# wangrui2025/GDKVM

Hardware: AMD Instinct MI355X
Metric: frames/sec (GDKVM forward + argmax mask), EchoNet 112x112x32 clips (higher is better)
Workload: dtype bf16; 1 GPU; BASELINE.json configs[1]: EchoNet-Dynamic 112x112x32 bf16 inference, batch=16 per GPU; clips_per_gpu=16, frames_per_clip=32, image=112x112, heads=1, key_dim=64, rule=delta_sequential, world_size=1, ranks_seen=1

## Files before the change

### gdkvm_amd/csrc/conv3x3_tile.hip

```cpp
#include <atomic>
#include "gdkvm_device.hpp"

namespace {

constexpr int CT_CK = 64;
constexpr int CT_PIX = 160;
constexpr int CT_SLOTS = CT_PIX / 16;
constexpr int CT_MAXMT = 13;
constexpr int CT_VARIANT_128 = 4, CT_VARIANT_64 = 3;

struct ConvTileArgs {
    const bf16_t* x; const bf16_t* w; const float* bias; const bf16_t* res; bf16_t* y;
    const bf16_t* x2; int C1;
    int N, H, W, C, K;
    int fpt, th, tiles_y, ntiles;
    int bw, bh, band_px, npieces;
    int relu;
    float inv_band, inv_bw, inv_tw, inv_w;
    int perm;
};

__host__ __device__ __forceinline__ int ct_channel(int kt, int j, int perm)
{
    return perm ? 32 * (kt >> 1) + 8 * (j >> 2) + 4 * (kt & 1) + (j & 3) : 16 * kt + j;
}

template <int NWN, int NTW, bool PK, int NWV = 8, int MAXMT = CT_MAXMT>
__global__ __launch_bounds__(64 * NWV, (NWV == 4 ? 2 : 1)) void conv3x3_tile_kernel(ConvTileArgs a)
{
    constexpr int MW = NWV / NWN, MTW = (MAXMT + MW - 1) / MW;
    extern __shared__ __attribute__((aligned(16))) unsigned char ct_band[];
    const int tid = threadIdx.x, lane = tid & 63, li = lane & 15, g = lane >> 4;
    const int w = __builtin_amdgcn_readfirstlane(tid >> 6), wn = w % NWN, wm = w / NWN;
    const int H = a.H, W = a.W, C = a.C, K = a.K, BW = a.bw;
    const int band_bytes = a.npieces * 1024, nchunk = C / CT_CK;
    const int tpix = a.fpt * a.th * W;
    const int co0 = blockIdx.y * (16 * NTW * NWN) + 16 * NTW * wn;

    f32x4 bias4[NTW];
#pragma unroll
    for (int nt = 0; nt < NTW; ++nt) {
        const int kt = min(co0 / 16 + nt, K / 16 - 1);
        const float* bp = a.bias + ct_channel(kt, 4 * g, a.perm);
        asm volatile("global_load_dwordx4 %0, %1, off" : "=&v"(bias4[nt]) : "v"(bp) : "memory");
    }

    constexpr int PP = NWV == 8 ? 7 : 8;
    const int cs1 = a.C1, cs2 = a.x2 ? C - a.C1 : C;
    unsigned g_off1[PP], g_off2[PP];
#pragma unroll
    for (int u = 0; u < PP; ++u) {
        const int j = w + NWV * u, d = 64 * j + lane, pix = d / CT_SLOTS, c = d - CT_SLOTS * pix;
        const int f = idx_div(pix, a.inv_band), r = pix - f * (a.bh * BW), by = idx_div(r, a.inv_bw), bx = r - by * BW;
        const int sp = (f * H + by - 1) * W + bx - 1;
        const bool live = j < a.npieces && c < 8 && pix < a.band_px && bx >= 1 && bx <= W && (a.tiles_y > 1 || (by >= 1 && by <= a.th));
        g_off1[u] = live ? (unsigned)(sp * cs1 * 2 + c * 16) : RSRC_DEAD;
        g_off2[u] = live ? (unsigned)(sp * cs2 * 2 + c * 16) : RSRC_DEAD;
    }
    const unsigned lds0 = (unsigned)reinterpret_cast<uintptr_t>(ct_band);
    const int nlive = max(0, (a.npieces - w + NWV - 1) / NWV);
    struct Geo { int px0, npx, row0; };
    auto geo_of = [&](int tile) __attribute__((always_inline)) {
        const int ty = tile % a.tiles_y, fg = tile / a.tiles_y;
        Geo q;
        q.px0 = fg * a.fpt * H * W;
        q.npx = min(a.fpt, a.N - fg * a.fpt) * H * W;
        q.row0 = ty * a.th * W;
        return q;
    };
    auto fetch = [&](const Geo q, int chunk, int buf) __attribute__((always_inline)) {
        const bool second = a.x2 != nullptr && chunk * CT_CK >= a.C1;
        const int cs = second ? cs2 : cs1;
        const bf16_t* base = (second ? a.x2 : a.x) + (long long)q.px0 * cs;
        const __amdgpu_buffer_rsrc_t rsrc = make_rsrc(base, q.npx * cs * 2);
        const unsigned ts = (unsigned)((q.row0 * cs + chunk * CT_CK - (second ? a.C1 : 0)) * 2);
        const unsigned dst0 = lds0 + buf * band_bytes + 1024 * w;
#pragma unroll
        for (int u = 0; u < PP; ++u) {
            const unsigned dst = u < nlive ? dst0 + 1024 * NWV * u : lds0 + 2 * band_bytes;
            __builtin_amdgcn_raw_ptr_buffer_load_lds(rsrc, lds_dma_dst(dst), 16,
                                                     (int)((second ? g_off2[u] : g_off1[u]) + ts), 0, 0, 0);
        }
    };

    int tile = blockIdx.x;
    Geo cur = geo_of(min(tile, a.ntiles - 1));
    if (tile < a.ntiles) fetch(cur, 0, 0);

    unsigned pbase[MTW];
#pragma unroll
    for (int m = 0; m < MTW; ++m) {
        const int p = min(16 * (wm + MW * m) + li, tpix - 1);
        const int f = idx_div(p, a.inv_tw), r = p - f * (a.th * W), py = idx_div(r, a.inv_w), px = r - py * W;
        pbase[m] = (unsigned)(((f * a.bh + py) * BW + px) * CT_PIX + g * 16);
    }
    const bf16_t* wrow[NTW];
// ... 27 lines not shown
    constexpr int WD = 3, KU = 6;
    WF wr[WD];
#pragma unroll
    for (int j = 0; j < WD; ++j) wload(wr[j], j);
    for (; tile < a.ntiles; tile += gridDim.x) {
        const Geo nxt = geo_of(min(tile + (int)gridDim.x, a.ntiles - 1));
        f32x4 acc[MTW][NTW];
#pragma unroll
        for (int m = 0; m < MTW; ++m)
#pragma unroll
            for (int nt = 0; nt < NTW; ++nt) acc[m][nt] = f32x4{0.f, 0.f, 0.f, 0.f};
        for (int chunk = 0; chunk < nchunk; ++chunk, ++gc) {
            const int buf = gc & 1;
            asm volatile("s_waitcnt vmcnt(%0) lgkmcnt(0)" ::"n"(WD * NTW) : "memory");
            asm volatile("s_barrier" ::: "memory");
            {
                const bool more = chunk + 1 < nchunk;
                Geo q;
                q.px0 = more ? cur.px0 : nxt.px0; q.npx = more ? cur.npx : nxt.npx; q.row0 = more ? cur.row0 : nxt.row0;
                fetch(q, more ? chunk + 1 : 0, buf ^ 1);
            }
            const unsigned char* band = ct_band + buf * band_bytes;
            auto load_x = [&](bf16x8 (&xb)[MTW], int r) __attribute__((always_inline)) {
                r = min(r, 17);
                const int tap = r >> 1, kh = r & 1, dy = tap / 3, dx = tap - 3 * dy;
                const unsigned off = (unsigned)((dy * BW + dx) * CT_PIX + kh * 64);
#pragma unroll
                for (int m = 0; m < MTW; ++m) {
                    xb[m] = *reinterpret_cast<const bf16x8*>(band + pbase[m] + off);
                }
            };
            auto mfmas = [&](const bf16x8 (&xb)[MTW], const WF& wfr) __attribute__((always_inline)) {
#pragma unroll
                for (int m = 0; m < MTW; ++m)
// ... 218 lines not shown
}

namespace {
template <int NWN, int NTW, int NWV = 8, int MAXMT = CT_MAXMT>
void launch_tile(bool packed, dim3 grid, size_t lds, hipStream_t st, const ConvTileArgs& a)
{
    if (packed) hipLaunchKernelGGL((conv3x3_tile_kernel<NWN, NTW, true, NWV, MAXMT>), grid, dim3(64 * NWV), lds, st, a);
    else hipLaunchKernelGGL((conv3x3_tile_kernel<NWN, NTW, false, NWV, MAXMT>), grid, dim3(64 * NWV), lds, st, a);
}
template <int NWN, int NTW, int NWV = 8, int MAXMT = CT_MAXMT>
bool setattr_tile()
{
    return hipFuncSetAttribute(reinterpret_cast<const void*>(conv3x3_tile_kernel<NWN, NTW, true, NWV, MAXMT>), hipFuncAttributeMaxDynamicSharedMemorySize, 113 * 1024) == hipSuccess
        && hipFuncSetAttribute(reinterpret_cast<const void*>(conv3x3_tile_kernel<NWN, NTW, false, NWV, MAXMT>), hipFuncAttributeMaxDynamicSharedMemorySize, 113 * 1024) == hipSuccess;
}
}

int gdkvm_conv3x3_tile_launch(const void* x, const void* x2, int C1, const void* w, const float* bias, const void* residual, void* y,
                              int N, int C, int H, int W, int K, int relu, int variant, int packed, hipStream_t st)
{
    if (variant == 0 && K % 128 == 0 && CT_VARIANT_128 == 4) {
        if (gdkvm_conv3x3_tile_launch(x, x2, C1, w, bias, residual, y, N, C, H, W, K, relu, 4, packed, st) == 0) return 0;
        variant = 2;
    }
    if (variant == 0 && K % 128 != 0 && (H * W <= 16 * 7 || 2 * W <= 16 * 7)) {
        if (gdkvm_conv3x3_tile_launch(x, x2, C1, w, bias, residual, y, N, C, H, W, K, relu, 5, packed, st) == 0) return 0;
        variant = 3;
    }
    if (C % CT_CK || K % 16 || W > 64 || W < 1 || H < 1 || N < 1 || variant < 0 || variant > 5) return 1;
    if (variant == 4 && K % 128) return 1;
    const bool half = variant == 4 || variant == 5;
    if (x2 && (C1 <= 0 || C1 >= C || C1 % CT_CK)) return 1;
    ConvTileArgs a;
    a.x2 = static_cast<const bf16_t*>(x2); a.C1 = x2 ? C1 : C;
    a.x = static_cast<const bf16_t*>(x); a.w = static_cast<const bf16_t*>(w); a.bias = bias;
    a.res = static_cast<const bf16_t*>(residual); a.y = static_cast<bf16_t*>(y);
    a.N = N; a.H = H; a.W = W; a.C = C; a.K = K; a.relu = relu;
    const int maxpix = half ? 16 * 7 : 16 * CT_MAXMT;
    const int maxpieces = half ? 32 : 56;
    if (H * W <= maxpix) { a.th = H; a.fpt = maxpix / (H * W); a.tiles_y = 1; if (a.fpt > N) a.fpt = N; }
    else { a.fpt = 1; a.th = maxpix / W; if (a.th < 1) return 1; a.tiles_y = (H + a.th - 1) / a.th; }
    a.bw = W + 2; a.bh = a.th + 2;
    auto pieces = [&]() { a.band_px = a.fpt * a.bh * a.bw; return (a.band_px * CT_SLOTS + 63) / 64; };
    while (pieces() > maxpieces && a.fpt > 1) --a.fpt;
    while (pieces() > maxpieces && a.th > 1) { --a.th; a.bh = a.th + 2; a.tiles_y = (H + a.th - 1) / a.th; }
    a.npieces = pieces();
    if (a.npieces > maxpieces) return 1;
    if ((long long)(a.fpt * H + 2) * W * (x2 ? (C1 > C - C1 ? C1 : C - C1) : C) * 2 >= 0x7fffffffLL) return 1;
    a.inv_band = 1.0f / (float)(a.bh * a.bw); a.inv_bw = 1.0f / (float)a.bw;
    a.inv_tw = 1.0f / (float)(a.th * W); a.inv_w = 1.0f / (float)W;
    a.perm = K % 32 == 0;
    const long long groups = (N + a.fpt - 1) / a.fpt;
    const long long ntiles = groups * a.tiles_y;
    if (ntiles <= 0 || ntiles > 0x7fffffffLL) return 1;
    a.ntiles = (int)ntiles;
    if (variant == 0) variant = K % 128 == 0 ? 2 : CT_VARIANT_64;
    const int kwg = (variant == 2 || variant == 4) ? 128 : 64;
    const int gy = (K + kwg - 1) / kwg;
    const size_t lds = (size_t)2 * a.npieces * 1024 + 1024;
    int per = (half ? 512 : 256) / gy; if (per < 1) per = 1;
    const int gx = (int)(ntiles < per ? ntiles : per);
    static std::atomic<unsigned long long> done_mask{0};
    int dev = 0;
    if (hipGetDevice(&dev) != hipSuccess) return 1;
    const unsigned long long bit = 1ull << (dev & 63);
    if (!(done_mask.load(std::memory_order_relaxed) & bit)) {
        if (!setattr_tile<4, 1>() || !setattr_tile<4, 2>() || !setattr_tile<2, 2>() || !setattr_tile<4, 2, 4, 7>() || !setattr_tile<2, 2, 4, 7>()) return 1;
        done_mask.fetch_or(bit, std::memory_order_relaxed);
    }
    switch (variant) {
// ... 9 lines not shown
```

### gdkvm_amd/csrc/conv_dispatch.hip

```cpp
#include "gdkvm_common.hpp"

int gdkvm_conv3x3_c64_launch(const void* x, const void* w, const float* bias, const void* residual, void* y, int N, int H, int W,
                             int relu, int packed, hipStream_t st);
int gdkvm_conv3x3_tile_launch(const void* x, const void* x2, int C1, const void* w, const float* bias, const void* residual, void* y,
                              int N, int C, int H, int W, int K, int relu, int variant, int packed, hipStream_t st);
int gdkvm_conv_igemm_launch(const void* x, const void* wpacked, const float* bias, const void* residual, void* y,
                            int N, int C, int H, int W, int K, int R, int S, int stride, int pad, int relu,
                            const void* w2packed, const float* bias2, void* y2, hipStream_t st);

extern "C" int gdkvm_conv_bias_act(const void* x, const void* w, const float* bias, const void* residual, void* y,
                                   int N, int C, int H, int W, int K, int R, int S, int stride, int pad, int relu, int kernel,
                                   int io_dtype, void* stream)
{
    if (io_dtype != GDKVM_BF16) return gdkvm_fail(GDKVM_ERR_DTYPE, "conv_bias_act: only bf16 is implemented");
    if (N < 0 || C <= 0 || H <= 0 || W <= 0 || K <= 0 || R <= 0 || S <= 0 || stride <= 0 || pad < 0 || C % 8 || K % 8
        || H + 2 * pad < R || W + 2 * pad < S)
        return gdkvm_fail(GDKVM_ERR_SHAPE, "conv_bias_act: N=%d C=%d H=%d W=%d K=%d %dx%d stride %d pad %d (C, K multiples of 8)",
                          N, C, H, W, K, R, S, stride, pad);
    const bool packed = kernel & GDKVM_CONV_PACKED_WEIGHTS;
    kernel &= ~GDKVM_CONV_PACKED_WEIGHTS;
    if (kernel != 0 && (kernel < 4 || kernel > 11)) return gdkvm_fail(GDKVM_ERR_ARG, "conv_bias_act: kernel=%d (0 = by shape, 4, 5, 6..8, 9, 10, 11)", kernel);
    if (kernel == 9) {
        if (!packed) return gdkvm_fail(GDKVM_ERR_ARG, "conv_bias_act: kernel 9 reads the gdkvm_conv_igemm_pack_weights copy of the weights (flag %d)", GDKVM_CONV_PACKED_WEIGHTS);
        if (C % 32 || K % 128) return gdkvm_fail(GDKVM_ERR_SHAPE, "conv_bias_act: kernel 9 needs C a multiple of 32 and K of 128 (C=%d K=%d)", C, K);
// ... 45 lines not shown
        return gdkvm_fail(GDKVM_ERR_SHAPE, "conv_cat_bias_act: N=%d C1=%d C2=%d H=%d W=%d K=%d (C1, C2 multiples of 64, K of 16)", N, C1, C2, H, W, K);
    if (N == 0) return GDKVM_OK;
    if (!x1 || !x2 || !w || !bias || !y) return gdkvm_fail(GDKVM_ERR_ARG, "conv_cat_bias_act: null pointer");
    if (!gdkvm_aligned16(x1) || !gdkvm_aligned16(x2) || !gdkvm_aligned16(w) || !gdkvm_aligned16(y) || !gdkvm_aligned16(bias) || (residual && !gdkvm_aligned16(residual)))
        return gdkvm_fail(GDKVM_ERR_ARG, "conv_cat_bias_act: pointers must be 16-byte aligned");
    if ((size_t)N * H * W * (C1 + C2) >= (1ull << 31) || (size_t)N * H * W * K >= (1ull << 31))
        return gdkvm_fail(GDKVM_ERR_SHAPE, "conv_cat_bias_act: tensor too large for 32-bit offsets");
    if (int rc = gdkvm_check_device()) return rc;
    if (gdkvm_conv3x3_tile_launch(x1, x2, C1, w, bias, residual, y, N, C1 + C2, H, W, K, relu, kernel >= 10 ? kernel - 6 : (kernel >= 6 ? kernel - 5 : 0), packed ? 1 : 0,
                                  static_cast<hipStream_t>(stream)))
        return gdkvm_fail(GDKVM_ERR_SHAPE, "conv_cat_bias_act: %dx%d is not served (rows of at most 64 pixels)", H, W);
    GDKVM_LAUNCH_CHECK("conv3x3_tile_kernel");
    return GDKVM_OK;
}

extern "C" int gdkvm_conv_down_bias_act(const void* x, const void* w, const float* bias, void* y, int relu,
                                        const void* w_down, const float* bias_down, void* y_down,
                                        int N, int C, int H, int W, int K, int R, int S, int stride, int pad, int io_dtype, void* stream)
{
    if (io_dtype != GDKVM_BF16) return gdkvm_fail(GDKVM_ERR_DTYPE, "conv_down_bias_act: only bf16 is implemented");
    if (N < 0 || C <= 0 || H <= 0 || W <= 0 || K <= 0 || R <= 0 || S != R || !(R & 1) || stride <= 0 || pad != R / 2 || C % 32 || K % 128)
        return gdkvm_fail(GDKVM_ERR_SHAPE, "conv_down_bias_act: N=%d C=%d H=%d W=%d K=%d %dx%d stride %d pad %d (odd square window, pad = R/2, "
                                           "C a multiple of 32, K of 128)", N, C, H, W, K, R, S, stride, pad);
    if (N == 0) return GDKVM_OK;
    if (!x || !w || !bias || !y || !w_down || !y_down) return gdkvm_fail(GDKVM_ERR_ARG, "conv_down_bias_act: null pointer");
    const void* ptrs[] = {x, w, bias, y, w_down, y_down};
    for (const void* p : ptrs) if (!gdkvm_aligned16(p)) return gdkvm_fail(GDKVM_ERR_ARG, "conv_down_bias_act: pointers must be 16-byte aligned");
    if (bias_down && !gdkvm_aligned16(bias_down)) return gdkvm_fail(GDKVM_ERR_ARG, "conv_down_bias_act: pointers must be 16-byte aligned");
    if (int rc = gdkvm_check_device()) return rc;
    if (gdkvm_conv_igemm_launch(x, w, bias, nullptr, y, N, C, H, W, K, R, S, stride, pad, relu, w_down, bias_down, y_down, static_cast<hipStream_t>(stream)))
// ... 5 lines not shown
```

### gdkvm_amd/csrc/gdkvm_device.hpp

```cpp
#pragma once
#include <type_traits>

#include "gdkvm_common.hpp"

typedef float f32x2 __attribute__((ext_vector_type(2)));
typedef unsigned u32x4 __attribute__((ext_vector_type(4)));

template <int I, int E, class F>
__device__ __forceinline__ void static_for(F&& f)
{
    if constexpr (I < E) {
        f(std::integral_constant<int, I>{});
        static_for<I + 1, E>(f);
    }
}

__device__ __forceinline__ int idx_div(int n, float inv) { return (int)(((float)n + 0.5f) * inv); }

__device__ __forceinline__ unsigned pack_bf16x2(float a, float b) { return (unsigned)f32_to_bf16(a) | ((unsigned)f32_to_bf16(b) << 16); }
__device__ __forceinline__ uint2 pack_bf16x4(const f32x4& v) { return make_uint2(pack_bf16x2(v[0], v[1]), pack_bf16x2(v[2], v[3])); }
__device__ __forceinline__ uint4 pack_bf16x8(const float (&v)[8])
{
    uint4 o;
    o.x = pack_bf16x2(v[0], v[1]);
// ... 12 lines not shown
    const unsigned w[4] = {u.x, u.y, u.z, u.w};
#pragma unroll
    for (int j = 0; j < 4; ++j) { v[2 * j] = bf16_lo(w[j]); v[2 * j + 1] = bf16_hi(w[j]); }
}

typedef __attribute__((address_space(3))) void* lds_dst_t;
__device__ __forceinline__ lds_dst_t lds_dma_dst(const void* p) { return reinterpret_cast<lds_dst_t>(reinterpret_cast<uintptr_t>(p)); }
__device__ __forceinline__ lds_dst_t lds_dma_dst(unsigned addr) { return reinterpret_cast<lds_dst_t>(static_cast<uintptr_t>(addr)); }

constexpr int RSRC_WORD3 = 0x00020000;
__device__ __forceinline__ __amdgpu_buffer_rsrc_t make_rsrc(const void* p, int bytes)
{
    return __builtin_amdgcn_make_buffer_rsrc(const_cast<void*>(p), 0, bytes, RSRC_WORD3);
}
constexpr unsigned RSRC_DEAD = 0x80000000u;
```

### gdkvm_amd/model.py

```python
from __future__ import annotations

from dataclasses import dataclass
import os
from typing import NamedTuple, Optional, Tuple

import torch
import torch.nn as nn
import torch.nn.functional as F

from . import ops

_RULES = {"gated_linear": ops.RULE_GATED_LINEAR, "delta_parallel": ops.RULE_DELTA_PARALLEL,
          "delta_sequential": ops.RULE_DELTA_SEQUENTIAL}

_KEY_REMAP: dict = {}


@dataclass
class GDKVMConfig:
    in_channels: int = 3
    num_classes: int = 2
    heads: int = 1
    key_dim: int = 64
    value_dim: int = 256
# ... 223 lines not shown
    buf = torch.empty((x.shape[0], padded), dtype=x.dtype, device=x.device)
    buf[:, :n].copy_(x.reshape(x.shape[0], n))
    return buf[:, :n].unflatten(1, x.shape[1:]) if x.dim() > 2 else buf[:, :n]


class UpBlock(nn.Module):
    def __init__(self, cin, cskip, cout):
        super().__init__()
        self.conv = nn.Sequential(nn.Conv2d(cin + cskip, cout, 3, 1, 1, bias=False), _bn(cout), nn.ReLU(inplace=True),
                                  nn.Conv2d(cout, cout, 3, 1, 1, bias=False), _bn(cout), nn.ReLU(inplace=True))

    def forward(self, x, skip):
        c = self.conv
        if (isinstance(c[0], FusedConv) and not torch.is_grad_enabled() and x.is_cuda and x.dtype == torch.bfloat16
                and skip.dtype == torch.bfloat16 and c[0].cat_served(x.shape[1], skip.shape[1], skip.shape[-1])):
            u = ops.upsample_bilinear(x.contiguous(memory_format=torch.channels_last), skip.shape[2:])
            y = c[0].forward_cat(u, skip)
            for m in list(c)[1:]:
                y = m(y)
            return y
        if (x.is_cuda and x.dtype == torch.bfloat16 and skip.dtype == torch.bfloat16
                and x.shape[1] % 8 == 0 and skip.shape[1] % 8 == 0):
            x = ops.upsample_cat(x.contiguous(memory_format=torch.channels_last),
                                 skip.contiguous(memory_format=torch.channels_last))
        else:
            x = torch.cat([F.interpolate(x, size=skip.shape[-2:], mode="bilinear", align_corners=False), skip], 1)
        if len(c) == 6 and isinstance(c[1], nn.BatchNorm2d):
            return _bn_act(c[4], _conv(c[3], _bn_act(c[1], _conv(c[0], x), True)), True)
        return c(x)


class HeadFeature(NamedTuple):
# ... 74 lines not shown
                and d.conv.out_channels == cv.out_channels and cv.in_channels % 32 == 0 and cv.out_channels % 128 == 0
                and cv.weight.dtype == torch.bfloat16 and d.conv.weight.dtype == torch.bfloat16
                and cv.weight.is_contiguous(memory_format=torch.channels_last)
                and self._tile(cv.in_channels, cv.out_channels, cv.stride[0], False, x.shape[-1]) is None):
            return None
        dw = d.conv.weight if d.conv.weight.is_contiguous(memory_format=torch.channels_last) else d.conv.weight.contiguous(memory_format=torch.channels_last)
        return ops.conv_down_bias_act(x.contiguous(memory_format=torch.channels_last), cv.weight, self.epi.bias, self._packed(x.device, igemm=True),
                                      dw, d._packed(x.device, igemm=True), None, cv.stride[0], self.relu)

    def cat_served(self, c1: int, c2: int, width: int) -> bool:
        cv = self.conv
        return (not getattr(self, "bias_folded_downstream", False) and cv.kernel_size == (3, 3) and cv.groups == 1
                and cv.dilation == (1, 1) and cv.stride == (1, 1) and cv.padding == (1, 1) and cv.weight.is_cuda
                and cv.weight.dtype == torch.bfloat16 and cv.weight.is_contiguous(memory_format=torch.channels_last)
                and c1 % 64 == 0 and c2 % 64 == 0 and c1 + c2 == cv.in_channels and cv.out_channels % 16 == 0 and width <= 64)

    def forward_cat(self, x1, x2):
        cl = torch.channels_last
        return ops.conv_cat_bias_act(x1.contiguous(memory_format=cl), x2.contiguous(memory_format=cl), self.conv.weight, self.epi.bias,
                                     None, self.relu, 0, self._packed(x1.device))

    def forward(self, x, residual=None):
        cv = self.conv
        folded = getattr(self, "bias_folded_downstream", False)
        if (not folded and x.is_cuda and x.dtype == torch.bfloat16 and cv.kernel_size == (3, 3) and cv.groups == 1
                and cv.dilation == (1, 1) and cv.stride[0] == cv.stride[1] and cv.padding == (1, 1) and cv.weight.dtype == torch.bfloat16
                and cv.in_channels % 8 == 0 and cv.out_channels % 8 == 0 and cv.weight.is_contiguous(memory_format=torch.channels_last)):
            tile = self._tile(cv.in_channels, cv.out_channels, cv.stride[0], residual is not None, x.shape[-1])
            if tile is not None:
                packed = self._packed(x.device) if tile in (4, 5) else None
# ... 810 lines not shown
```

### gdkvm_amd/ops.py

```python
from __future__ import annotations

import contextlib
import ctypes
import math
import os
from typing import Optional, Tuple

import torch

RULE_GATED_LINEAR, RULE_DELTA_PARALLEL, RULE_DELTA_SEQUENTIAL = 0, 1, 2
FLAG_NORMALIZE_QK, FLAG_GATE_LOGITS, FLAG_TRAIN, FLAG_WIDE_RANGE = 1, 2, 4, 8


def recurrence_flags(rule: int, flags: int) -> int:
    return flags | FLAG_WIDE_RANGE if rule == RULE_DELTA_PARALLEL else flags
F32, BF16 = 0, 1

_PKG = os.path.dirname(os.path.abspath(__file__))
_SO = os.path.join(_PKG, "libgdkvm_hip.so")
_lib = None
_vp, _sz, _i = ctypes.c_void_p, ctypes.c_size_t, ctypes.c_int

SIGNATURES = {
    "gdkvm_abi_version": (_i, []),
# ... 42 lines not shown
    "gdkvm_head_bwd": (_i, [_vp] * 7 + [_sz] + [_i] * 6 + [_vp]),
    "gdkvm_proj_rows": (_i, [_vp] * 6 + [ctypes.c_longlong] + [_i] * 5 + [_vp]),
    "gdkvm_stem_conv_pool": (_i, [_vp] * 4 + [_i] * 4 + [_vp]),
    "gdkvm_stem_conv_pool_nchw": (_i, [_vp] * 4 + [_i] * 5 + [_vp]),
    "gdkvm_stem_conv_nchw": (_i, [_vp] * 3 + [_i] * 5 + [_vp]),
    "gdkvm_stem_pack_s2d": (_i, [_vp, _vp, _i] + [ctypes.c_longlong] * 4 + [_vp]),
    "gdkvm_stem_wgrad_workspace_bytes": (_sz, [_i] * 3),
    "gdkvm_stem_wgrad_nchw": (_i, [_vp] * 3 + [ctypes.c_longlong] * 4 + [_vp, _sz] + [_i] * 5 + [_vp]),
    "gdkvm_gate_logits": (_i, [_vp] * 7 + [_i] * 5 + [_vp]),
    "gdkvm_proj_gates": (_i, [_vp] * 13 + [_i] * 7 + [_vp]),
    "gdkvm_conv_bias_act": (_i, [_vp] * 5 + [_i] * 12 + [_vp]),
    "gdkvm_conv3x3_pack_weights": (_i, [_vp, _vp, _i, _i, _i, _vp]),
    "gdkvm_conv_igemm_pack_weights": (_i, [_vp, _vp, _i, _i, _i, _i, _i, _vp]),
    "gdkvm_conv_down_bias_act": (_i, [_vp] * 4 + [_i] + [_vp] * 3 + [_i] * 10 + [_vp]),
    "gdkvm_conv_cat_bias_act": (_i, [_vp] * 6 + [_i] * 9 + [_vp]),
    "gdkvm_conv_s2_dgrad_pack_bytes": (_sz, [_i] * 3),
    "gdkvm_conv_s2_pack_train": (_i, [_vp] * 7 + [_i, _i, _vp]),
    "gdkvm_conv_s2_dgrad": (_i, [_vp] * 4 + [_i] * 7 + [_vp]),
    "gdkvm_conv_wgrad_strided_workspace_bytes": (_sz, [_i] * 9),
    "gdkvm_conv_wgrad_strided": (_i, [_vp] * 3 + [ctypes.c_longlong] * 4 + [_vp, _sz] + [_i] * 10 + [_vp]),
    "gdkvm_conv3x3_pack_weights_dgrad": (_i, [_vp, _vp, _i, _i, _i, _vp]),
    "gdkvm_conv3x3_pack_weights_train": (_i, [_i, _vp, _vp, _vp, _vp, _vp, _vp, _vp]),
    "gdkvm_conv3x3_wgrad_workspace_bytes": (_sz, [_i] * 5),
    "gdkvm_conv3x3_wgrad": (_i, [_vp, _vp, _vp, _vp, _sz] + [_i] * 6 + [_vp]),
    "gdkvm_conv3x3_wgrad_krsc": (_i, [_vp, _vp, _vp, _vp, _sz] + [_i] * 6 + [_vp]),
    "gdkvm_upsample_cat": (_i, [_vp] * 3 + [_i] * 8 + [_vp]),
    "gdkvm_upsample_cat_bwd": (_i, [_vp] * 3 + [_i] * 8 + [_vp]),
    "gdkvm_bias_relu_maxpool": (_i, [_vp] * 3 + [_i] * 7 + [_vp]),
    "gdkvm_stem_s2d": (_i, [_vp] * 2 + [_i] * 6 + [_vp]),
    "gdkvm_upsample_argmax_dice": (_i, [_vp] * 4 + [_i] * 7 + [_vp]),
# ... 1116 lines not shown
    n, c, hh, ww = x.shape
    out = torch.empty((n, cpad, hh // 2, ww // 2), device=x.device, dtype=x.dtype, memory_format=torch.channels_last)
    _call("gdkvm_stem_s2d", x.device, x, out, n, c, hh, ww, cpad, _io_dtype(x))
    return out


def upsample_bilinear(lo: torch.Tensor, size) -> torch.Tensor:
    _channels_last("upsample_bilinear", lo, dtype=torch.bfloat16, shape="[N,C,h,w]")
    n, c1, hl, wl = lo.shape
    H, W = int(size[0]), int(size[1])
    out = torch.empty((n, c1, H, W), dtype=lo.dtype, device=lo.device, memory_format=torch.channels_last)
    _call("gdkvm_upsample_cat", lo.device, lo, None, out, n, hl, wl, H, W, c1, 0, BF16)
    return out


def conv_cat_bias_act(x1: torch.Tensor, x2: torch.Tensor, weight: torch.Tensor, bias: torch.Tensor,
                      residual: Optional[torch.Tensor] = None, relu: bool = True, tile: int = 0,
                      packed: Optional[torch.Tensor] = None) -> torch.Tensor:
    _channels_last("conv_cat_bias_act", x1, x2, dtype=torch.bfloat16)
    n, c1, hh, ww = x1.shape
    c2 = x2.shape[1]
    if tuple(x2.shape) != (n, c2, hh, ww):
        raise GdkvmError("conv_cat_bias_act: x1 and x2 must agree in batch and size")
    if weight.dim() != 4 or weight.dtype != torch.bfloat16 or tuple(weight.shape[1:]) != (c1 + c2, 3, 3) or \
            not weight.is_contiguous(memory_format=torch.channels_last):
        raise GdkvmError("conv_cat_bias_act: weight must be channels_last bf16 [K,C1+C2,3,3]")
    k = weight.shape[0]
    if bias.dtype != torch.float32 or bias.numel() != k:
        raise GdkvmError("bias must be float32 [K]")
    y = torch.empty((n, k, hh, ww), dtype=x1.dtype, device=x1.device, memory_format=torch.channels_last)
    if residual is not None and (residual.shape != y.shape or residual.dtype != y.dtype or
                                 not residual.is_contiguous(memory_format=torch.channels_last)):
        raise GdkvmError("residual must match the output (shape, dtype, channels_last)")
    if packed is not None:
        if packed.dtype != torch.bfloat16 or packed.numel() != weight.numel() or packed.device != x1.device:
            raise GdkvmError("conv_cat_bias_act: packed must be conv3x3_pack_weights(weight)")
        tile |= CONV_PACKED_WEIGHTS
    _call("gdkvm_conv_cat_bias_act", x1.device, x1, x2, packed if packed is not None else weight, bias, residual, y,
          n, c1, c2, hh, ww, k, int(relu), tile, BF16)
    return y


def _upsample_cat_fwd(lo: torch.Tensor, skip: torch.Tensor) -> torch.Tensor:
    _channels_last("upsample_cat", lo, skip)
    if lo.dtype != torch.bfloat16 or skip.dtype != torch.bfloat16 or lo.shape[0] != skip.shape[0]:
        raise GdkvmError("upsample_cat: bf16 tensors with equal batch")
    n, c1, hl, wl = lo.shape
    _, c2, H, W = skip.shape
    out = torch.empty((n, c1 + c2, H, W), dtype=lo.dtype, device=lo.device, memory_format=torch.channels_last)
    _call("gdkvm_upsample_cat", lo.device, lo, skip, out, n, hl, wl, H, W, c1, c2, BF16)
    return out


def stem_conv_pool(xs: torch.Tensor, w_s2d: torch.Tensor, bias: torch.Tensor) -> torch.Tensor:
# ... 531 lines not shown
```

### include/gdkvm.h

```cpp
#ifndef GDKVM_H
#define GDKVM_H

#include <stddef.h>
#include <stdint.h>

#ifdef __cplusplus
extern "C" {
#endif

#define GDKVM_ABI_VERSION 1

enum { GDKVM_OK = 0, GDKVM_ERR_SHAPE = -1, GDKVM_ERR_DTYPE = -2, GDKVM_ERR_ARCH = -3,
       GDKVM_ERR_LAUNCH = -4, GDKVM_ERR_WORKSPACE = -5, GDKVM_ERR_ARG = -6,
       GDKVM_ERR_RANGE = -7  };

enum { GDKVM_F32 = 0, GDKVM_BF16 = 1 };

enum { GDKVM_RULE_GATED_LINEAR = 0,
       GDKVM_RULE_DELTA_PARALLEL = 1,
       GDKVM_RULE_DELTA_SEQUENTIAL = 2    };

enum { GDKVM_FLAG_NORMALIZE_QK = 1,
       GDKVM_FLAG_GATE_LOGITS = 2,
       GDKVM_FLAG_TRAIN = 4,
// ... 156 lines not shown
                        int io_dtype, void* stream);
int gdkvm_conv_down_bias_act(const void* x, const void* w, const float* bias, void* y, int relu,
                             const void* w_down, const float* bias_down, void* y_down,
                             int N, int C, int H, int W, int K, int R, int S, int stride, int pad, int io_dtype, void* stream);
size_t gdkvm_conv_s2_dgrad_pack_bytes(int C, int K, int with_down);
int gdkvm_conv_s2_pack_train(const float* w, const long long* w_strides, const float* w_down, const long long* w_down_strides,
                             void* packed_fwd, void* packed_fwd_down, void* packed_dgrad, int K, int C, void* stream);
int gdkvm_conv_s2_dgrad(const void* dy, const void* dy_down, const void* packed_dgrad, void* dx,
                        int N, int C, int H, int W, int K, int with_down, int io_dtype, void* stream);
size_t gdkvm_conv_wgrad_strided_workspace_bytes(int N, int C, int H, int W, int K, int R, int S, int stride, int pad);
int gdkvm_conv_wgrad_strided(const void* x, const void* dy, float* dw, long long sk, long long sc, long long sr, long long ss,
                             void* workspace, size_t workspace_bytes,
                             int N, int C, int H, int W, int K, int R, int S, int stride, int pad, int io_dtype, void* stream);
int gdkvm_conv_cat_bias_act(const void* x1, const void* x2, const void* w, const float* bias, const void* residual, void* y,
                            int N, int C1, int C2, int H, int W, int K, int relu, int kernel, int io_dtype, void* stream);

int gdkvm_bias_relu_maxpool(const void* x, const float* bias, void* y, int N, int H, int W, int C,
                            int x_rows, int x_cols, int io_dtype, void* stream);

int gdkvm_stem_conv_pool(const void* xs, const void* w, const float* bias, void* y, int N, int Hs, int Ws,
                         int io_dtype, void* stream);
int gdkvm_stem_conv_pool_nchw(const void* x, const void* w, const float* bias, void* y, int N, int C, int H, int W,
                              int io_dtype, void* stream);
int gdkvm_stem_conv_nchw(const void* x, const void* w4, void* y, int N, int C, int H, int W, int io_dtype, void* stream);
int gdkvm_stem_pack_s2d(const float* w7, void* w4, int C, long long sk, long long sc, long long sr, long long ss, void* stream);
size_t gdkvm_stem_wgrad_workspace_bytes(int N, int H, int W);
int gdkvm_stem_wgrad_nchw(const void* x, const void* dy, float* dw, long long sk, long long sc, long long sr, long long ss,
                          void* workspace, size_t workspace_bytes, int N, int C, int H, int W, int io_dtype, void* stream);

int gdkvm_maxpool_fwd(const void* x, void* y, void* idx, int N, int H, int W, int C, int io_dtype, void* stream);
// ... 52 lines not shown
```

Before: 654,700 frames/s.

## Fuse 2x bilinear upsample into the concat 3x3 conv tile kernel

Adds an UP variant of the tiled 3x3 conv kernel that DMA-stages low-resolution rows into LDS and bilinearly upsamples them into the conv band in-kernel, instead of writing a separate upsampled tensor to global memory and reading it back. The decoder's upsample+cat+conv path uses this by default (env GDKVM_UPCAT_FUSED). This removes one kernel launch and the full-resolution intermediate traffic, at the cost of extra LDS, an extra barrier per chunk of the first input, and interpolation ALU work inside the conv loop.

```diff
diff --git a/gdkvm_amd/csrc/conv3x3_tile.hip b/gdkvm_amd/csrc/conv3x3_tile.hip
--- a/gdkvm_amd/csrc/conv3x3_tile.hip
+++ b/gdkvm_amd/csrc/conv3x3_tile.hip
@@ -19,14 +19,21 @@
     float inv_band, inv_bw, inv_tw, inv_w;
     int perm;
 };
+struct ConvUpArgs : ConvTileArgs {
+    int hl, wl, nlr;
+    int stage_px, nstage;
+    int stage_off;
+    int nrp;
+    float inv_slr, inv_wl, inv_ncp, inv_nrp;
+};
 
 __host__ __device__ __forceinline__ int ct_channel(int kt, int j, int perm)
 {
     return perm ? 32 * (kt >> 1) + 8 * (j >> 2) + 4 * (kt & 1) + (j & 3) : 16 * kt + j;
 }
 
-template <int NWN, int NTW, bool PK, int NWV = 8, int MAXMT = CT_MAXMT>
-__global__ __launch_bounds__(64 * NWV, (NWV == 4 ? 2 : 1)) void conv3x3_tile_kernel(ConvTileArgs a)
+template <int NWN, int NTW, bool PK, int NWV = 8, int MAXMT = CT_MAXMT, bool UP = false>
+__global__ __launch_bounds__(64 * NWV, (NWV == 4 ? 2 : 1)) void conv3x3_tile_kernel(std::conditional_t<UP, ConvUpArgs, ConvTileArgs> a)
 {
     constexpr int MW = NWV / NWN, MTW = (MAXMT + MW - 1) / MW;
     extern __shared__ __attribute__((aligned(16))) unsigned char ct_band[];
@@ -56,30 +63,50 @@
         const bool live = j < a.npieces && c < 8 && pix < a.band_px && bx >= 1 && bx <= W && (a.tiles_y > 1 || (by >= 1 && by <= a.th));
         g_off1[u] = live ? (unsigned)(sp * cs1 * 2 + c * 16) : RSRC_DEAD;
         g_off2[u] = live ? (unsigned)(sp * cs2 * 2 + c * 16) : RSRC_DEAD;
+        if constexpr (UP) {
+            const int spx = d >> 3, c8 = d & 7;
+            const int sf = idx_div(spx, a.inv_slr), sr = spx - sf * (a.nlr * a.wl), lr = idx_div(sr, a.inv_wl), lx = sr - lr * a.wl;
+            g_off1[u] = j < a.nstage && spx < a.stage_px ? (unsigned)((((sf * a.hl + lr) * a.wl + lx) * cs1 + c8 * 8) * 2) : RSRC_DEAD;
+        }
     }
     const unsigned lds0 = (unsigned)reinterpret_cast<uintptr_t>(ct_band);
     const int nlive = max(0, (a.npieces - w + NWV - 1) / NWV);
-    struct Geo { int px0, npx, row0; };
+    int nlive_up = 0, stage_off = 0;
+    if constexpr (UP) { nlive_up = max(0, (a.nstage - w + NWV - 1) / NWV); stage_off = a.stage_off; }
+    struct Geo { int px0, npx, row0, r0, lr0, nfr; };
     auto geo_of = [&](int tile) __attribute__((always_inline)) {
         const int ty = tile % a.tiles_y, fg = tile / a.tiles_y;
         Geo q;
         q.px0 = fg * a.fpt * H * W;
         q.npx = min(a.fpt, a.N - fg * a.fpt) * H * W;
         q.row0 = ty * a.th * W;
+        q.r0 = q.lr0 = q.nfr = 0;
+        if constexpr (UP) {
+            q.r0 = ty * a.th; q.lr0 = max((q.r0 - 2) >> 1, 0); q.nfr = min(a.fpt, a.N - fg * a.fpt);
+        }
         return q;
     };
     auto fetch = [&](const Geo q, int chunk, int buf) __attribute__((always_inline)) {
         const bool second = a.x2 != nullptr && chunk * CT_CK >= a.C1;
         const int cs = second ? cs2 : cs1;
-        const bf16_t* base = (second ? a.x2 : a.x) + (long long)q.px0 * cs;
-        const __amdgpu_buffer_rsrc_t rsrc = make_rsrc(base, q.npx * cs * 2);
-        const unsigned ts = (unsigned)((q.row0 * cs + chunk * CT_CK - (second ? a.C1 : 0)) * 2);
-        const unsigned dst0 = lds0 + buf * band_bytes + 1024 * w;
+        const bool up = UP && !second;
+        const bf16_t* base = (second ? a.x2 : a.x) + (long long)(up ? q.px0 >> 2 : q.px0) * cs;
+        const __amdgpu_buffer_rsrc_t rsrc = make_rsrc(base, (up ? q.npx >> 2 : q.npx) * cs * 2);
+        unsigned ts = (unsigned)((q.row0 * cs + chunk * CT_CK - (second ? a.C1 : 0)) * 2);
+        unsigned dst0 = lds0 + buf * band_bytes + 1024 * w;
+        int nl = nlive;
+        if constexpr (UP) {
+            ts = up ? (unsigned)((q.lr0 * (W >> 1) * cs + chunk * CT_CK) * 2) : ts;
+            dst0 = up ? lds0 + stage_off + 1024 * w : dst0;
+            nl = up ? nlive_up : nlive;
+        }
 #pragma unroll
         for (int u = 0; u < PP; ++u) {
-            const unsigned dst = u < nlive ? dst0 + 1024 * NWV * u : lds0 + 2 * band_bytes;
-            __builtin_amdgcn_raw_ptr_buffer_load_lds(rsrc, lds_dma_dst(dst), 16,
-                                                     (int)((second ? g_off2[u] : g_off1[u]) + ts), 0, 0, 0);
+            const unsigned dst = u < nl ? dst0 + 1024 * NWV * u : lds0 + 2 * band_bytes;
+            unsigned go;
+            if constexpr (UP) go = g_off1[u] ^ ((g_off1[u] ^ g_off2[u]) & (second ? ~0u : 0u));
+            else go = second ? g_off2[u] : g_off1[u];
+            __builtin_amdgcn_raw_ptr_buffer_load_lds(rsrc, lds_dma_dst(dst), 16, (int)(go + ts), 0, 0, 0);
         }
     };
 
@@ -137,10 +164,52 @@
             const int buf = gc & 1;
             asm volatile("s_waitcnt vmcnt(%0) lgkmcnt(0)" ::"n"(WD * NTW) : "memory");
             asm volatile("s_barrier" ::: "memory");
+            if constexpr (UP) if (chunk * CT_CK < a.C1) {
+                const unsigned stg = lds0 + stage_off;
+                unsigned char* const bandw = ct_band + buf * band_bytes;
+                const int hl = H >> 1, wl = W >> 1, ncp = wl + 1, ip0 = (cur.r0 - 2) >> 1;
+                const int nitems = a.fpt * a.nrp * ncp * 8;
+#pragma unroll 1
+                for (int i = tid; i < nitems; i += 64 * NWV) {
+                    const int c8 = i & 7, t = i >> 3;
+                    const int t2 = idx_div(t, a.inv_ncp), jp = t - t2 * ncp - 1, f = idx_div(t2, a.inv_nrp), ip = ip0 + t2 - f * a.nrp;
+                    const int y0 = 2 * ip + 1, x0o = 2 * jp + 1;
+                    const int by0 = y0 - cur.r0 + 1;
+                    const bool vy[2] = {y0 >= 0 && y0 < H, y0 + 1 >= 0 && y0 + 1 < H}, vx[2] = {x0o >= 0, x0o + 1 < W};
+                    u32x4 o[2][2] = {};
+                    if ((vy[0] || vy[1]) && f < cur.nfr) {
+                        const int ra = max(ip, 0) - cur.lr0, rb = min(ip + 1, hl - 1) - cur.lr0;
+                        const int xa_ = max(jp, 0), xb_ = min(jp + 1, wl - 1);
+                        const unsigned s0 = stg + (f * a.nlr + ra) * wl * 128 + c8 * 16, s1 = stg + (f * a.nlr + rb) * wl * 128 + c8 * 16;
+                        u32x4 t00, t01, t10, t11;
+                        asm volatile("ds_read_b128 %0, %1" : "=&v"(t00) : "v"(s0 + xa_ * 128) : "memory");
+                        asm volatile("ds_read_b128 %0, %1" : "=&v"(t01) : "v"(s0 + xb_ * 128) : "memory");
+                        asm volatile("ds_read_b128 %0, %1" : "=&v"(t10) : "v"(s1 + xa_ * 128) : "memory");
+                        asm volatile("ds_read_b128 %0, %1" : "=&v"(t11) : "v"(s1 + xb_ * 128) : "memory");
+                        asm volatile("s_waitcnt lgkmcnt(0)" : "+v"(t00), "+v"(t01), "+v"(t10), "+v"(t11) :: "memory");
+                        const float ly[2] = {0.25f, y0 + 1 == 0 ? 0.f : 0.75f}, hy[2] = {0.75f, 1.f - ly[1]};
+                        bilerp2x_bf16x8(t00, t01, t10, t11, hy, ly, o);
+                    }
+#pragma unroll
+                    for (int ey = 0; ey < 2; ++ey) {
+                        if (by0 + ey < 0 || by0 + ey >= a.bh) continue;
+                        const bool rowin = vy[ey] && f < cur.nfr;
+#pragma unroll
+                        for (int e = 0; e < 2; ++e) {
+                            const u32x4 z = {0u, 0u, 0u, 0u};
+                            *reinterpret_cast<u32x4*>(bandw + ((f * a.bh + by0 + ey) * BW + x0o + 1 + e) * CT_PIX + c8 * 16) = rowin && vx[e] ? o[ey][e] : z;
+                        }
+                    }
+                }
+                asm volatile("s_waitcnt lgkmcnt(0)" ::: "memory");
+                asm volatile("s_barrier" ::: "memory");
+            }
             {
                 const bool more = chunk + 1 < nchunk;
                 Geo q;
                 q.px0 = more ? cur.px0 : nxt.px0; q.npx = more ? cur.npx : nxt.npx; q.row0 = more ? cur.row0 : nxt.row0;
+                q.r0 = q.lr0 = q.nfr = 0;
+                if constexpr (UP) q.lr0 = more ? cur.lr0 : nxt.lr0;
                 fetch(q, more ? chunk + 1 : 0, buf ^ 1);
             }
             const unsigned char* band = ct_band + buf * band_bytes;
@@ -389,6 +458,71 @@
     return hipFuncSetAttribute(reinterpret_cast<const void*>(conv3x3_tile_kernel<NWN, NTW, true, NWV, MAXMT>), hipFuncAttributeMaxDynamicSharedMemorySize, 113 * 1024) == hipSuccess
         && hipFuncSetAttribute(reinterpret_cast<const void*>(conv3x3_tile_kernel<NWN, NTW, false, NWV, MAXMT>), hipFuncAttributeMaxDynamicSharedMemorySize, 113 * 1024) == hipSuccess;
 }
+constexpr size_t CT_UP_LDS = 80 * 1024;
+template <int NWN, int NTW>
+bool setattr_up()
+{
+    return hipFuncSetAttribute(reinterpret_cast<const void*>(conv3x3_tile_kernel<NWN, NTW, true, 4, 7, true>), hipFuncAttributeMaxDynamicSharedMemorySize, (int)CT_UP_LDS) == hipSuccess;
+}
+
+bool tile_geometry(ConvTileArgs& a, int maxpix, int maxpieces)
+{
+    const int N = a.N, H = a.H, W = a.W;
+    if (H * W <= maxpix) { a.th = H; a.fpt = maxpix / (H * W); a.tiles_y = 1; if (a.fpt > N) a.fpt = N; }
+    else { a.fpt = 1; a.th = maxpix / W; if (a.th < 1) return false; a.tiles_y = (H + a.th - 1) / a.th; }
+    a.bw = W + 2; a.bh = a.th + 2;
+    auto pieces = [&]() { a.band_px = a.fpt * a.bh * a.bw; return (a.band_px * CT_SLOTS + 63) / 64; };
+    while (pieces() > maxpieces && a.fpt > 1) --a.fpt;
+    while (pieces() > maxpieces && a.th > 1) { --a.th; a.bh = a.th + 2; a.tiles_y = (H + a.th - 1) / a.th; }
+    a.npieces = pieces();
+    if (a.npieces > maxpieces) return false;
+    a.inv_band = 1.0f / (float)(a.bh * a.bw); a.inv_bw = 1.0f / (float)a.bw;
+    a.inv_tw = 1.0f / (float)(a.th * W); a.inv_w = 1.0f / (float)W;
+    const long long groups = (N + a.fpt - 1) / a.fpt;
+    const long long ntiles = groups * a.tiles_y;
+    if (ntiles <= 0 || ntiles > 0x7fffffffLL) return false;
+    a.ntiles = (int)ntiles;
+    return true;
+}
+}
+
+int gdkvm_conv3x3_upcat_launch(const void* lo, const void* x2, int C1, const void* w, const float* bias, const void* residual, void* y,
+                               int N, int C, int H, int W, int K, int relu, hipStream_t st)
+{
+    if (C % CT_CK || K % 16 || W > 64 || W < 2 || H < 2 || (H | W) & 1 || N < 1 || !x2 || C1 <= 0 || C1 >= C || C1 % CT_CK) return 1;
+    ConvUpArgs a;
+    a.x2 = static_cast<const bf16_t*>(x2); a.C1 = C1;
+    a.x = static_cast<const bf16_t*>(lo); a.w = static_cast<const bf16_t*>(w); a.bias = bias;
+    a.res = static_cast<const bf16_t*>(residual); a.y = static_cast<bf16_t*>(y);
+    a.N = N; a.H = H; a.W = W; a.C = C; a.K = K; a.relu = relu;
+    if (!tile_geometry(a, 16 * 7, 32)) return 1;
+    if ((long long)(a.fpt * H + 2) * W * (C1 > C - C1 ? C1 : C - C1) * 2 >= 0x7fffffffLL) return 1;
+    a.perm = K % 32 == 0;
+    a.hl = H / 2; a.wl = W / 2;
+    a.nlr = a.bh / 2 + 2 < a.hl ? a.bh / 2 + 2 : a.hl;
+    a.stage_px = a.fpt * a.nlr * a.wl;
+    a.nstage = (a.stage_px + 7) / 8;
+    if (a.nstage > 32) return 1;
+    a.inv_slr = 1.0f / (float)(a.nlr * a.wl); a.inv_wl = 1.0f / (float)a.wl;
+    a.nrp = a.bh / 2 + 1; a.inv_ncp = 1.0f / (float)(a.wl + 1); a.inv_nrp = 1.0f / (float)a.nrp;
+    a.stage_off = 2 * a.npieces * 1024 + 1024;
+    const size_t lds = (size_t)a.stage_off + (size_t)a.nstage * 1024;
+    if (lds > CT_UP_LDS) return 1;
+    const int kwg = K % 128 == 0 ? 128 : 64;
+    const int gy = (K + kwg - 1) / kwg;
+    int per = 512 / gy; if (per < 1) per = 1;
+    const int gx = a.ntiles < per ? a.ntiles : per;
+    static std::atomic<unsigned long long> done_mask{0};
+    int dev = 0;
+    if (hipGetDevice(&dev) != hipSuccess) return 1;
+    const unsigned long long bit = 1ull << (dev & 63);
+    if (!(done_mask.load(std::memory_order_relaxed) & bit)) {
+        if (!setattr_up<4, 2>() || !setattr_up<2, 2>()) return 1;
+        done_mask.fetch_or(bit, std::memory_order_relaxed);
+    }
+    if (kwg == 128) hipLaunchKernelGGL((conv3x3_tile_kernel<4, 2, true, 4, 7, true>), dim3(gx, gy), dim3(256), lds, st, a);
+    else hipLaunchKernelGGL((conv3x3_tile_kernel<2, 2, true, 4, 7, true>), dim3(gx, gy), dim3(256), lds, st, a);
+    return 0;
 }
 
 int gdkvm_conv3x3_tile_launch(const void* x, const void* x2, int C1, const void* w, const float* bias, const void* residual, void* y,
@@ -413,22 +547,10 @@
     a.N = N; a.H = H; a.W = W; a.C = C; a.K = K; a.relu = relu;
     const int maxpix = half ? 16 * 7 : 16 * CT_MAXMT;
     const int maxpieces = half ? 32 : 56;
-    if (H * W <= maxpix) { a.th = H; a.fpt = maxpix / (H * W); a.tiles_y = 1; if (a.fpt > N) a.fpt = N; }
-    else { a.fpt = 1; a.th = maxpix / W; if (a.th < 1) return 1; a.tiles_y = (H + a.th - 1) / a.th; }
-    a.bw = W + 2; a.bh = a.th + 2;
-    auto pieces = [&]() { a.band_px = a.fpt * a.bh * a.bw; return (a.band_px * CT_SLOTS + 63) / 64; };
-    while (pieces() > maxpieces && a.fpt > 1) --a.fpt;
-    while (pieces() > maxpieces && a.th > 1) { --a.th; a.bh = a.th + 2; a.tiles_y = (H + a.th - 1) / a.th; }
-    a.npieces = pieces();
-    if (a.npieces > maxpieces) return 1;
+    if (!tile_geometry(a, maxpix, maxpieces)) return 1;
     if ((long long)(a.fpt * H + 2) * W * (x2 ? (C1 > C - C1 ? C1 : C - C1) : C) * 2 >= 0x7fffffffLL) return 1;
-    a.inv_band = 1.0f / (float)(a.bh * a.bw); a.inv_bw = 1.0f / (float)a.bw;
-    a.inv_tw = 1.0f / (float)(a.th * W); a.inv_w = 1.0f / (float)W;
     a.perm = K % 32 == 0;
-    const long long groups = (N + a.fpt - 1) / a.fpt;
-    const long long ntiles = groups * a.tiles_y;
-    if (ntiles <= 0 || ntiles > 0x7fffffffLL) return 1;
-    a.ntiles = (int)ntiles;
+    const long long ntiles = a.ntiles;
     if (variant == 0) variant = K % 128 == 0 ? 2 : CT_VARIANT_64;
     const int kwg = (variant == 2 || variant == 4) ? 128 : 64;
     const int gy = (K + kwg - 1) / kwg;
diff --git a/gdkvm_amd/csrc/conv_dispatch.hip b/gdkvm_amd/csrc/conv_dispatch.hip
--- a/gdkvm_amd/csrc/conv_dispatch.hip
+++ b/gdkvm_amd/csrc/conv_dispatch.hip
@@ -4,6 +4,8 @@
                              int relu, int packed, hipStream_t st);
 int gdkvm_conv3x3_tile_launch(const void* x, const void* x2, int C1, const void* w, const float* bias, const void* residual, void* y,
                               int N, int C, int H, int W, int K, int relu, int variant, int packed, hipStream_t st);
+int gdkvm_conv3x3_upcat_launch(const void* lo, const void* x2, int C1, const void* w, const float* bias, const void* residual, void* y,
+                               int N, int C, int H, int W, int K, int relu, hipStream_t st);
 int gdkvm_conv_igemm_launch(const void* x, const void* wpacked, const float* bias, const void* residual, void* y,
                             int N, int C, int H, int W, int K, int R, int S, int stride, int pad, int relu,
                             const void* w2packed, const float* bias2, void* y2, hipStream_t st);
@@ -83,6 +85,29 @@
     return GDKVM_OK;
 }
 
+extern "C" int gdkvm_conv_upcat_bias_act(const void* lo, const void* x2, const void* w, const float* bias, const void* residual, void* y,
+                                         int N, int C1, int C2, int H, int W, int K, int relu, int kernel, int io_dtype, void* stream)
+{
+    if (io_dtype != GDKVM_BF16) return gdkvm_fail(GDKVM_ERR_DTYPE, "conv_upcat_bias_act: only bf16 is implemented");
+    if (kernel != GDKVM_CONV_PACKED_WEIGHTS)
+        return gdkvm_fail(GDKVM_ERR_ARG, "conv_upcat_bias_act: kernel=%d (%d: the gdkvm_conv3x3_pack_weights copy of the weights, wave grid by shape)", kernel, GDKVM_CONV_PACKED_WEIGHTS);
+    if (N < 0 || C1 <= 0 || C2 <= 0 || C1 % 64 || C2 % 64 || H <= 0 || W <= 0 || K <= 0 || K % 16)
+        return gdkvm_fail(GDKVM_ERR_SHAPE, "conv_upcat_bias_act: N=%d C1=%d C2=%d H=%d W=%d K=%d (C1, C2 multiples of 64, K of 16)", N, C1, C2, H, W, K);
+    if (H % 2 || W % 2 || W > 64)
+        return gdkvm_fail(GDKVM_ERR_SHAPE, "conv_upcat_bias_act: H=%d W=%d (an exact 2x enlargement: both even; rows of at most 64 pixels)", H, W);
+    if (N == 0) return GDKVM_OK;
+    if (!lo || !x2 || !w || !bias || !y) return gdkvm_fail(GDKVM_ERR_ARG, "conv_upcat_bias_act: null pointer");
+    if (!gdkvm_aligned16(lo) || !gdkvm_aligned16(x2) || !gdkvm_aligned16(w) || !gdkvm_aligned16(y) || !gdkvm_aligned16(bias) || (residual && !gdkvm_aligned16(residual)))
+        return gdkvm_fail(GDKVM_ERR_ARG, "conv_upcat_bias_act: pointers must be 16-byte aligned");
+    if ((size_t)N * H * W * (C1 + C2) >= (1ull << 31) || (size_t)N * H * W * K >= (1ull << 31))
+        return gdkvm_fail(GDKVM_ERR_SHAPE, "conv_upcat_bias_act: tensor too large for 32-bit offsets");
+    if (int rc = gdkvm_check_device()) return rc;
+    if (gdkvm_conv3x3_upcat_launch(lo, x2, C1, w, bias, residual, y, N, C1 + C2, H, W, K, relu, static_cast<hipStream_t>(stream)))
+        return gdkvm_fail(GDKVM_ERR_SHAPE, "conv_upcat_bias_act: %dx%d is not served (the band and the staged rows of a tile must fit 80 KB of LDS)", H, W);
+    GDKVM_LAUNCH_CHECK("conv3x3_tile_kernel");
+    return GDKVM_OK;
+}
+
 extern "C" int gdkvm_conv_down_bias_act(const void* x, const void* w, const float* bias, void* y, int relu,
                                         const void* w_down, const float* bias_down, void* y_down,
                                         int N, int C, int H, int W, int K, int R, int S, int stride, int pad, int io_dtype, void* stream)
diff --git a/gdkvm_amd/csrc/gdkvm_device.hpp b/gdkvm_amd/csrc/gdkvm_device.hpp
--- a/gdkvm_amd/csrc/gdkvm_device.hpp
+++ b/gdkvm_amd/csrc/gdkvm_device.hpp
@@ -50,3 +50,35 @@
     return __builtin_amdgcn_make_buffer_rsrc(const_cast<void*>(p), 0, bytes, RSRC_WORD3);
 }
 constexpr unsigned RSRC_DEAD = 0x80000000u;
+
+__device__ __forceinline__ void bilerp2x_bf16x8(const u32x4& a, const u32x4& b, const u32x4& c, const u32x4& d,
+                                                const float (&hy)[2], const float (&ly)[2], u32x4 (&o)[2][2])
+{
+#pragma clang fp contract(off)
+#pragma unroll
+    for (int q = 0; q < 4; ++q) {
+        float v[2][2][2];
+#pragma unroll
+        for (int h = 0; h < 2; ++h) {
+            const float A = h ? bf16_hi(a[q]) : bf16_lo(a[q]), B = h ? bf16_hi(b[q]) : bf16_lo(b[q]);
+            const float C = h ? bf16_hi(c[q]) : bf16_lo(c[q]), D = h ? bf16_hi(d[q]) : bf16_lo(d[q]);
+#pragma unroll
+            for (int e = 0; e < 2; ++e) {
+                const float lx = e ? 0.75f : 0.25f, hx = e ? 0.25f : 0.75f;
+                if (q & 1) {
+                    const float top = __fmaf_rn(hx, A, __fmul_rn(lx, B)), bot = __fmaf_rn(hx, C, __fmul_rn(lx, D));
+#pragma unroll
+                    for (int ey = 0; ey < 2; ++ey) v[ey][e][h] = __fmaf_rn(hy[ey], top, __fmul_rn(ly[ey], bot));
+                } else {
+                    const float top = __fmaf_rn(lx, B, __fmul_rn(hx, A)), bot = __fmaf_rn(lx, D, __fmul_rn(hx, C));
+#pragma unroll
+                    for (int ey = 0; ey < 2; ++ey) v[ey][e][h] = __fmaf_rn(ly[ey], bot, __fmul_rn(hy[ey], top));
+                }
+            }
+        }
+#pragma unroll
+        for (int ey = 0; ey < 2; ++ey)
+#pragma unroll
+            for (int e = 0; e < 2; ++e) o[ey][e][q] = pack_bf16x2(v[ey][e][0], v[ey][e][1]);
+    }
+}
diff --git a/gdkvm_amd/model.py b/gdkvm_amd/model.py
--- a/gdkvm_amd/model.py
+++ b/gdkvm_amd/model.py
@@ -261,8 +261,11 @@
         c = self.conv
         if (isinstance(c[0], FusedConv) and not torch.is_grad_enabled() and x.is_cuda and x.dtype == torch.bfloat16
                 and skip.dtype == torch.bfloat16 and c[0].cat_served(x.shape[1], skip.shape[1], skip.shape[-1])):
-            u = ops.upsample_bilinear(x.contiguous(memory_format=torch.channels_last), skip.shape[2:])
-            y = c[0].forward_cat(u, skip)
+            if c[0].upcat_served(x.shape[1], skip.shape[1], tuple(x.shape[2:]), tuple(skip.shape[2:])):
+                y = c[0].forward_upcat(x, skip)
+            else:
+                u = ops.upsample_bilinear(x.contiguous(memory_format=torch.channels_last), skip.shape[2:])
+                y = c[0].forward_cat(u, skip)
             for m in list(c)[1:]:
                 y = m(y)
             return y
@@ -367,6 +370,15 @@
                 and cv.dilation == (1, 1) and cv.stride == (1, 1) and cv.padding == (1, 1) and cv.weight.is_cuda
                 and cv.weight.dtype == torch.bfloat16 and cv.weight.is_contiguous(memory_format=torch.channels_last)
                 and c1 % 64 == 0 and c2 % 64 == 0 and c1 + c2 == cv.in_channels and cv.out_channels % 16 == 0 and width <= 64)
+
+    def upcat_served(self, c1: int, c2: int, lo_size, size) -> bool:
+        return (os.environ.get("GDKVM_UPCAT_FUSED", "1") != "0" and self.cat_served(c1, c2, size[1])
+                and size == (2 * lo_size[0], 2 * lo_size[1]))
+
+    def forward_upcat(self, lo, x2):
+        cl = torch.channels_last
+        return ops.conv_upcat_bias_act(lo.contiguous(memory_format=cl), x2.contiguous(memory_format=cl), self.conv.weight, self.epi.bias,
+                                       None, self.relu, self._packed(lo.device))
 
     def forward_cat(self, x1, x2):
         cl = torch.channels_last
diff --git a/gdkvm_amd/ops.py b/gdkvm_amd/ops.py
--- a/gdkvm_amd/ops.py
+++ b/gdkvm_amd/ops.py
@@ -80,6 +80,7 @@
     "gdkvm_conv_igemm_pack_weights": (_i, [_vp, _vp, _i, _i, _i, _i, _i, _vp]),
     "gdkvm_conv_down_bias_act": (_i, [_vp] * 4 + [_i] + [_vp] * 3 + [_i] * 10 + [_vp]),
     "gdkvm_conv_cat_bias_act": (_i, [_vp] * 6 + [_i] * 9 + [_vp]),
+    "gdkvm_conv_upcat_bias_act": (_i, [_vp] * 6 + [_i] * 9 + [_vp]),
     "gdkvm_conv_s2_dgrad_pack_bytes": (_sz, [_i] * 3),
     "gdkvm_conv_s2_pack_train": (_i, [_vp] * 7 + [_i, _i, _vp]),
     "gdkvm_conv_s2_dgrad": (_i, [_vp] * 4 + [_i] * 7 + [_vp]),
@@ -1226,17 +1227,15 @@
     return out
 
 
-def conv_cat_bias_act(x1: torch.Tensor, x2: torch.Tensor, weight: torch.Tensor, bias: torch.Tensor,
-                      residual: Optional[torch.Tensor] = None, relu: bool = True, tile: int = 0,
-                      packed: Optional[torch.Tensor] = None) -> torch.Tensor:
-    _channels_last("conv_cat_bias_act", x1, x2, dtype=torch.bfloat16)
-    n, c1, hh, ww = x1.shape
-    c2 = x2.shape[1]
-    if tuple(x2.shape) != (n, c2, hh, ww):
-        raise GdkvmError("conv_cat_bias_act: x1 and x2 must agree in batch and size")
+def _conv_cat_operands(what: str, x1, x2, size, weight, bias, residual, packed) -> torch.Tensor:
+    _channels_last(what, x1, x2, dtype=torch.bfloat16)
+    n, c1 = x1.shape[:2]
+    c2, hh, ww = x2.shape[1:]
+    if x2.shape[0] != n or tuple(size) != (hh, ww):
+        raise GdkvmError(f"{what}: the two inputs must agree in batch and size")
     if weight.dim() != 4 or weight.dtype != torch.bfloat16 or tuple(weight.shape[1:]) != (c1 + c2, 3, 3) or \
             not weight.is_contiguous(memory_format=torch.channels_last):
-        raise GdkvmError("conv_cat_bias_act: weight must be channels_last bf16 [K,C1+C2,3,3]")
+        raise GdkvmError(f"{what}: weight must be channels_last bf16 [K,C1+C2,3,3]")
     k = weight.shape[0]
     if bias.dtype != torch.float32 or bias.numel() != k:
         raise GdkvmError("bias must be float32 [K]")
@@ -1244,12 +1243,33 @@
     if residual is not None and (residual.shape != y.shape or residual.dtype != y.dtype or
                                  not residual.is_contiguous(memory_format=torch.channels_last)):
         raise GdkvmError("residual must match the output (shape, dtype, channels_last)")
+    if packed is not None and (packed.dtype != torch.bfloat16 or packed.numel() != weight.numel() or packed.device != x1.device):
+        raise GdkvmError(f"{what}: packed must be conv3x3_pack_weights(weight)")
+    return y
+
+
+def conv_cat_bias_act(x1: torch.Tensor, x2: torch.Tensor, weight: torch.Tensor, bias: torch.Tensor,
+                      residual: Optional[torch.Tensor] = None, relu: bool = True, tile: int = 0,
+                      packed: Optional[torch.Tensor] = None) -> torch.Tensor:
+    y = _conv_cat_operands("conv_cat_bias_act", x1, x2, x1.shape[2:] if x1.dim() == 4 else (), weight, bias, residual, packed)
     if packed is not None:
-        if packed.dtype != torch.bfloat16 or packed.numel() != weight.numel() or packed.device != x1.device:
-            raise GdkvmError("conv_cat_bias_act: packed must be conv3x3_pack_weights(weight)")
         tile |= CONV_PACKED_WEIGHTS
+    n, c1, hh, ww = x1.shape
     _call("gdkvm_conv_cat_bias_act", x1.device, x1, x2, packed if packed is not None else weight, bias, residual, y,
-          n, c1, c2, hh, ww, k, int(relu), tile, BF16)
+          n, c1, x2.shape[1], hh, ww, y.shape[1], int(relu), tile, BF16)
+    return y
+
+
+def conv_upcat_bias_act(lo: torch.Tensor, x2: torch.Tensor, weight: torch.Tensor, bias: torch.Tensor,
+                        residual: Optional[torch.Tensor] = None, relu: bool = True,
+                        packed: Optional[torch.Tensor] = None) -> torch.Tensor:
+    size = (2 * lo.shape[2], 2 * lo.shape[3]) if lo.dim() == 4 else ()
+    y = _conv_cat_operands("conv_upcat_bias_act", lo, x2, size, weight, bias, residual, packed)
+    if packed is None:
+        packed = conv3x3_pack_weights(weight)
+    n, c1 = lo.shape[:2]
+    _call("gdkvm_conv_upcat_bias_act", lo.device, lo, x2, packed, bias, residual, y,
+          n, c1, x2.shape[1], size[0], size[1], y.shape[1], int(relu), CONV_PACKED_WEIGHTS, BF16)
     return y
 
 
diff --git a/include/gdkvm.h b/include/gdkvm.h
--- a/include/gdkvm.h
+++ b/include/gdkvm.h
@@ -194,6 +194,8 @@
                              int N, int C, int H, int W, int K, int R, int S, int stride, int pad, int io_dtype, void* stream);
 int gdkvm_conv_cat_bias_act(const void* x1, const void* x2, const void* w, const float* bias, const void* residual, void* y,
                             int N, int C1, int C2, int H, int W, int K, int relu, int kernel, int io_dtype, void* stream);
+int gdkvm_conv_upcat_bias_act(const void* lo, const void* x2, const void* w, const float* bias, const void* residual, void* y,
+                              int N, int C1, int C2, int H, int W, int K, int relu, int kernel, int io_dtype, void* stream);
 
 int gdkvm_bias_relu_maxpool(const void* x, const float* bias, void* y, int N, int H, int W, int C,
                             int x_rows, int x_cols, int io_dtype, void* stream);
```

Measured after the change: 661,400 frames/s (median of 6 runs). +1.0%, better.
